# MeteoSwiss/topo-descriptors

Measured on AMD Instinct MI355X. Metric: Mpixels/s (and % HBM roofline) per descriptor, 1/2/4/8 MI355X, higher is better.
Workload: dtype f32

## Files before the change

topo_descriptors_amd/csrc/disc_ring_wide_impl.hpp:

```cpp
#pragma once

#include "wide_classify.hpp"

namespace topo {

namespace {

constexpr int NCW = 6;

template <int SIZE>
struct WGeo {
    static constexpr DiscTable<SIZE> T = make_disc_table<SIZE>();
    static_assert(T.centre == 0 && T.off_min == -T.off_max, "odd disc sizes only");
    static constexpr int M = T.off_max;
    static constexpr int DL = (M + NCW - 1) / NCW;
    static constexpr int NVL = 64 - 2 * DL;
    static constexpr int TILE_W = NCW * NVL;
    static constexpr int X0 = NCW * DL;
    static constexpr int W = 64 * NCW;
    static constexpr int NR = T.num_runs;
    static_assert(NVL >= 16, "disc too wide for one wavefront");
    struct Sched {
        int first_step[SIZE];
        int order[SIZE];
        int centre_run;
    };
    static constexpr Sched make() {
        Sched t{};
        for (int r = 0; r < SIZE; ++r) t.first_step[r] = -1;
        for (int r = 0; r < SIZE; ++r) t.order[r] = 0;
        t.centre_run = -1;
        for (int D = 0; D <= DL; ++D)
            for (int s = 0; s < NCW; ++s)
                for (int q = 0; q < NCW; ++q) {
                    const int dr = NCW * D + s - q, dl = -NCW * D + s - q;
                    if (dr >= 0 && dr <= M) {
                        const int r = T.run_of[dr - T.off_min];
                        if (D > t.first_step[r]) t.first_step[r] = D;
                    }
                    if (dl < 0 && dl >= -M) {
                        const int r = T.run_of[dl - T.off_min];
                        if (D > t.first_step[r]) t.first_step[r] = D;
                    }
                }
        int n = 0;
        for (int D = DL; D >= 0; --D)
            for (int d = M; d >= 0; --d) {
                const int r = T.run_of[d - T.off_min];
                bool seen = false;
                for (int i = 0; i < n; ++i) seen = seen || t.order[i] == r;
                if (!seen && t.first_step[r] == D) t.order[n++] = r;
            }
        for (int r = 0; r < NR; ++r)
            if (T.run_lo[r] == 0 && T.run_hi[r] == 0) t.centre_run = r;
        return t;
    }
    static constexpr Sched S = make();
    static_assert(S.centre_run >= 0, "the disc's outermost column is the pixel's own row");
};

template <int SIZE>
struct WideCfg {
    using G = WGeo<SIZE>;
    static constexpr int SW = 3;
    static constexpr int CW = 8;
    static constexpr int NW = SW + CW;
    static constexpr int RPW = 2;
    static constexpr int B = CW * RPW;
    static constexpr int TH = 64;
    static constexpr int PPT = TH / B;
    static constexpr int R = SIZE + 2 * B;
    static constexpr int GR = 6;
    static constexpr int HALO = SIZE - 1;
    static constexpr int PAD = 1 + (B - (1 + HALO + B) % B) % B;
    static constexpr int PRO = PAD + HALO + B;
    static constexpr int NB_PRO = PRO / B;
    static constexpr size_t LDS = (size_t)(R + GR) * G::W * sizeof(uint32_t) + 2 * SW * sizeof(int) + 16;
    static_assert(SW * 128 == G::W, "two staged columns per staging lane");
    static_assert(TH % B == 0 && PRO % B == 0, "whole batches");
    static_assert(LDS <= 160 * 1024, "ring does not fit LDS");
    static_assert(NB_PRO <= 15, "batch history: two fields of a flag word");
};

constexpr bool tpi_wide_ring_fits(int size) {
    return size >= 5 && size % 2 == 1 && (size_t)(size + 32 + 6) * 384 * 4 + 64 <= 160 * 1024 && 64 - 2 * ((size / 2 + 5) / 6) >= 16;
}

template <int SIZE, int GR>
struct WPair {
    using G = WGeo<SIZE>;
    static constexpr int NR = G::NR;
    static constexpr int NK = 2 * G::M + 3;
    struct Tab {
        int rows;
        int nb;
        int kb[NK];
        int first[NK];
        int base[NK];
        int use[SIZE][2][2];
        int nload[SIZE];
        int load[SIZE][4];
    };
    static constexpr Tab make() {
        Tab t{};
        bool need[NK] = {};
        for (int i = 0; i < NR; ++i) {
            const int r = G::S.order[i];
            for (int w = 0; w < 2; ++w) {
                t.use[i][w][0] = G::T.run_hi[r] + 1 + G::M + w;
                t.use[i][w][1] = G::T.run_lo[r] + G::M + w;
            }
            for (int w = 0; w < 2; ++w)
                for (int e = 0; e < 2; ++e) {
                    const int k = t.use[i][w][e];
                    if (!need[k]) t.load[i][t.nload[i]++] = k;
                    need[k] = true;
                }
        }
        for (int k = 0; k < NK; ++k) {
            if (!need[k]) continue;
            ++t.rows;
            if (t.nb == 0 || k > t.kb[t.nb - 1] + GR) t.kb[t.nb++] = k;
            t.base[k] = t.nb - 1;
        }
        for (int b = 0; b < t.nb; ++b) t.first[b] = NR;
        for (int i = NR - 1; i >= 0; --i)
            for (int n = 0; n < t.nload[i]; ++n) t.first[t.base[t.load[i][n]]] = i;
        return t;
    }
    static constexpr Tab T = make();
    static constexpr bool check() {
        bool loaded[NK] = {};
        for (int i = 0; i < NR; ++i) {
            for (int n = 0; n < T.nload[i]; ++n) {
                const int k = T.load[i][n], b = T.base[k];
                if (k < T.kb[b] || k - T.kb[b] > GR || T.first[b] > i || loaded[k]) return false;
                loaded[k] = true;
            }
            for (int w = 0; w < 2; ++w)
                for (int e = 0; e < 2; ++e)
                    if (!loaded[T.use[i][w][e]]) return false;
        }
        return true;
    }
    static constexpr int kUnshared = 4 * NR;
    static_assert(check(), "every row loaded once, before its uses, within GR rows of a base formed by then");
    static_assert(T.rows < kUnshared, "the pair shares no prefix row");
    static_assert(SIZE != 67 || T.rows == 55, "67 px: 55 distinct prefix rows a pair (84 unshared)");
};

template <int N, int I = 0, class F>
__device__ __forceinline__ void wide_static_for(F&& f) {
    if constexpr (I < N) {
        f(std::integral_constant<int, I>{});
        wide_static_for<N, I + 1>(f);
    }
}

template <int SIZE>
struct WSweep {
    using G = WGeo<SIZE>;
    struct Tab {
        int firstR[G::DL + 1][NCW], firstL[G::DL + 1][NCW];
        int lo_s[G::NR][2][G::DL + 1][NCW], hi_s[G::NR][2][G::DL + 1][NCW];
    };
    static constexpr int tap(int side, int D, int s, int t) { return (side == 0 ? NCW * D : -NCW * D) + s - t; }
    static constexpr bool takes(int side, int di) { return side == 0 ? di >= 0 && di <= G::M : di < 0 && di >= -G::M; }
    static constexpr Tab make() {
        Tab t{};
        for (int D = 0; D <= G::DL; ++D)
            for (int o = 0; o < NCW; ++o) t.firstR[D][o] = t.firstL[D][o] = -1;
        for (int j = G::NR - 1; j >= 0; --j)
            for (int s = NCW - 1; s >= 0; --s)
                for (int D = 0; D <= G::DL; ++D)
                    for (int o = 0; o < NCW; ++o) {
                        const int dr = NCW * D + s - o, dl = -NCW * D + s - o;
                        if (dr >= 0 && dr <= G::M && G::T.run_of[dr - G::T.off_min] == G::S.order[j]) t.firstR[D][o] = j * NCW + s;
                        if (dl < 0 && dl >= -G::M && G::T.run_of[dl - G::T.off_min] == G::S.order[j]) t.firstL[D][o] = j * NCW + s;
                    }
        for (int j = 0; j < G::NR; ++j)
            for (int side = 0; side < 2; ++side)
                for (int D = 0; D <= G::DL; ++D)
                    for (int o = 0; o < NCW; ++o) {
                        int lo = NCW, hi = -1;
                        for (int s = 0; s < NCW; ++s) {
                            const int di = tap(side, D, s, o);
                            if (takes(side, di) && G::T.run_of[di - G::T.off_min] == G::S.order[j]) {
                                lo = s < lo ? s : lo;
                                hi = s;
                            }
                        }
                        t.lo_s[j][side][D][o] = lo;
                        t.hi_s[j][side][D][o] = hi;
                    }
        return t;
    }
    static constexpr Tab T = make();
    static constexpr bool covers() {
        int hits[NCW][2 * G::M + 1] = {};
        int total = 0;
        for (int j = 0; j < G::NR; ++j)
            for (int side = 0; side < 2; ++side)
                for (int D = 0; D <= G::DL; ++D)
                    for (int o = 0; o < NCW; ++o)
                        for (int s = T.lo_s[j][side][D][o]; s <= T.hi_s[j][side][D][o]; ++s) {
                            const int di = tap(side, D, s, o);
                            if (di < -G::M || di > G::M) return false;
                            ++hits[o][di + G::M];
                            ++total;
                        }
        for (int o = 0; o < NCW; ++o)
            for (int d = 0; d <= 2 * G::M; ++d)
                if (hits[o][d] != 1) return false;
        return total == NCW * (2 * G::M + 1);
    }
    static constexpr bool firsts_start_intervals() {
        for (int side = 0; side < 2; ++side)
            for (int D = 0; D <= G::DL; ++D)
                for (int o = 0; o < NCW; ++o) {
                    const int f = side == 0 ? T.firstR[D][o] : T.firstL[D][o];
                    for (int j = 0; j < G::NR; ++j) {
                        const bool empty = T.lo_s[j][side][D][o] > T.hi_s[j][side][D][o];
                        if (f < 0 || j < f / NCW) {
                            if (!empty) return false;
                        } else if (j == f / NCW) {
                            if (empty || T.lo_s[j][side][D][o] != f % NCW) return false;
                        }
                    }
                }
        return true;
    }
    static_assert(covers(), "the intervals take every tap of every output once: SIZE taps an output");
    static_assert(SIZE != 67 || NCW * (2 * G::M + 1) == 402, "67 px: 402 taps per side pair");
    static_assert(firsts_start_intervals(), "firstR / firstL name an interval's first column");
    static constexpr int prio_of(int D) { return 3 - (G::DL - D) * 4 / (G::DL + 1); }
};

#ifndef WIDE_LEAD
#define WIDE_LEAD 2
#endif
#ifndef WIDE_PRIO
#define WIDE_PRIO 1
#endif

#ifndef WIDE_STAMPS
#define WIDE_STAMPS 0
#endif
#ifndef WIDE_LEAN
#define WIDE_LEAN 1
#endif
#ifndef WIDE_STAGE_CEILING
#define WIDE_STAGE_CEILING 0
#endif
#if WIDE_STAMPS
constexpr int kWideStampBlocks = 2, kWideStampWaves = 11, kWideStampFields = 5;
__device__ unsigned long long wide_stamps[kWideStampBlocks][kWideStampWaves][kWideStampFields];
__device__ __forceinline__ uint32_t wide_now() {
    const uint32_t t = (uint32_t)__builtin_amdgcn_s_memtime();
    asm volatile("s_waitcnt lgkmcnt(0)" ::: "memory");
    return t;
}
#endif

typedef uint32_t u32x2w __attribute__((ext_vector_type(2)));
typedef __attribute__((address_space(3))) const char lds_char;
typedef __attribute__((address_space(1))) const u32x2w glb_u32x2w;
typedef __attribute__((address_space(3))) const volatile u32x2w lds_u32x2w;

template <int SIZE, int R, int GR, int LEAD, bool PRIO>
__device__ __forceinline__ void wide_pair_sum(const uint32_t* ring, int s0, int lane, uint32_t (&acc)[2][NCW], uint32_t (&ctr)[2][NCW]) {
    using G = WGeo<SIZE>;
    using PT = WPair<SIZE, GR>;
    using SW_ = WSweep<SIZE>;
    constexpr int NR = G::NR;
    constexpr int DL = G::DL;
    constexpr int M = G::M;
    constexpr uint32_t PB = (uint32_t)G::W * 4;
    constexpr uint32_t RB = (uint32_t)R * PB;
    u32x2w row[PT::NK][3];
    uint32_t pR[2][DL + 1][NCW], pL[2][DL + 1][NCW];
    uint32_t aR[2][NCW], aL[2][NCW];
    uint32_t vb[PT::T.nb];
    lds_char* q = (lds_char*)ring;
    const uint32_t b0 = (uint32_t)s0 * PB, lb = (uint32_t)lane * (NCW * 4);
    auto fetch = [&](auto I) {
        constexpr int i = decltype(I)::value;
#pragma unroll
        for (int b = 0; b < PT::T.nb; ++b)
            if (PT::T.first[b] == i) {
                const uint32_t d = b0 + (uint32_t)PT::T.kb[b] * PB;
                vb[b] = lb + min(d, d - RB);
                asm("" : "+v"(vb[b]));
            }
#pragma unroll
        for (int n = 0; n < PT::T.nload[i]; ++n) {
            const int k = PT::T.load[i][n];
            lds_char* pk = q + vb[PT::T.base[k]] + (uint32_t)(k - PT::T.kb[PT::T.base[k]]) * PB;
#pragma unroll
            for (int h = 0; h < 3; ++h) row[k][h] = *(lds_u32x2w*)(pk + 8 * h);
        }
    };
    auto close = [&](auto DD) {
        constexpr int D = decltype(DD)::value;
        wide_static_for<NCW * 2>([&](auto TW) {
            constexpr int t = decltype(TW)::value / 2, w = decltype(TW)::value % 2;
            constexpr bool anyr = SW_::T.firstR[D][t] >= 0, anyl = SW_::T.firstL[D][t] >= 0;
            uint32_t pr = 0, pl = 0;
            if constexpr (anyr) pr = pR[w][D][t];
            if constexpr (anyl) pl = pL[w][D][t];
            if constexpr (D == DL) {
                aR[w][t] = pr;
                aL[w][t] = pl;
            } else if constexpr (D == 0) {
                uint32_t own = anyr && anyl ? pr + pl : anyr ? pr : pl;
                asm("" : "+v"(own));
                own = hop_up(aL[w][t]) + own;
                asm("" : "+v"(own));
                aR[w][t] = hop(aR[w][t]) + own;
                asm("" : "+v"(aR[w][t]));
            } else {
                if constexpr (anyr) {
                    asm("" : "+v"(pr));
                    aR[w][t] = hop(aR[w][t]) + pr;
                } else {
                    aR[w][t] = hop(aR[w][t]);
                }
                if constexpr (anyl) {
                    asm("" : "+v"(pl));
                    aL[w][t] = hop_up(aL[w][t]) + pl;
                } else {
                    aL[w][t] = hop_up(aL[w][t]);
                }
            }
        });
        RING_SB();
    };
    wide_static_for<(LEAD < NR ? LEAD : NR)>([&](auto I) { fetch(I); });
    if constexpr (PRIO) CHAIN_SETPRIO(3);
    static_assert(DL >= 1 && G::S.first_step[G::S.order[0]] == DL, "the first run opens the chains, the last step (D = 0) closes both");
    wide_static_for<NR>([&](auto J) {
        constexpr int j = decltype(J)::value;
        constexpr int r = G::S.order[j];
        constexpr int D = G::S.first_step[r];
        constexpr int Dprev = j == 0 ? DL : G::S.first_step[G::S.order[j > 0 ? j - 1 : 0]];
        constexpr int Dnext = j + 1 < NR ? G::S.first_step[G::S.order[j + 1 < NR ? j + 1 : j]] : -1;
        if constexpr (PRIO && SW_::prio_of(D) != SW_::prio_of(Dprev)) CHAIN_SETPRIO(SW_::prio_of(D));
        if constexpr (j + LEAD < NR) fetch(std::integral_constant<int, j + LEAD>{});
        RING_SB();
        uint32_t cv[2][NCW], pre[2][NCW], suf[2][NCW];
#pragma unroll
        for (int w = 0; w < 2; ++w) {
#pragma unroll
            for (int s = 0; s < NCW; ++s) {
                cv[w][s] = row[PT::T.use[j][w][0]][s / 2][s % 2] - row[PT::T.use[j][w][1]][s / 2][s % 2];
                if (r == G::S.centre_run) ctr[w][s] = cv[w][s];
            }
            pre[w][0] = cv[w][0];
            suf[w][NCW - 1] = cv[w][NCW - 1];
#pragma unroll
            for (int s = 1; s < NCW; ++s) {
                pre[w][s] = pre[w][s - 1] + cv[w][s];
                suf[w][NCW - 1 - s] = suf[w][NCW - s] + cv[w][NCW - 1 - s];
            }
        }
        wide_static_for<2 * (DL + 1) * NCW>([&](auto ET) {
            constexpr int side = decltype(ET)::value / ((DL + 1) * NCW);
            constexpr int E = decltype(ET)::value / NCW % (DL + 1), t = decltype(ET)::value % NCW;
            constexpr int a = SW_::T.lo_s[j][side][E][t], b = SW_::T.hi_s[j][side][E][t];
            if constexpr (a <= b) {
                static_assert(E <= D, "a run arrives at the first step that takes it");
                constexpr bool starts = (side == 0 ? SW_::T.firstR[E][t] : SW_::T.firstL[E][t]) / NCW == j;
#pragma unroll
                for (int w = 0; w < 2; ++w) {
                    const uint32_t iv = a == b ? cv[w][a] : a == 0 ? pre[w][b] : b == NCW - 1 ? suf[w][a] :
                                        b == a + 1 ? cv[w][a] + cv[w][b] : pre[w][b] - pre[w][a - 1];
                    uint32_t& acc_p = side == 0 ? pR[w][E][t] : pL[w][E][t];
                    acc_p = starts ? iv : acc_p + iv;
                }
            }
        });
        RING_SB();
        wide_static_for<D - Dnext>([&](auto C) { close(std::integral_constant<int, D - decltype(C)::value>{}); });
    });
#pragma unroll
    for (int w = 0; w < 2; ++w)
#pragma unroll
        for (int t = 0; t < NCW; ++t) acc[w][t] = aR[w][t];
}


template <int SIZE>
__global__ __launch_bounds__(WideCfg<SIZE>::NW * 64) void tpi_ring_wide_kernel(WaveArgs p, int tiles_x, int tiles_y, PartRun deal) {
    using G = WGeo<SIZE>;
    using C = WideCfg<SIZE>;
    constexpr int B = C::B, R = C::R, PPT = C::PPT, SW = C::SW, NB_PRO = C::NB_PRO, DL = G::DL;
    constexpr unsigned kWindow = (1u << NB_PRO) - 1u;
    constexpr int kBad = 1, kFracOnly = 1 << 15;
    constexpr unsigned kHistMask = kWindow | kWindow * kFracOnly;
    extern __shared__ __attribute__((aligned(16))) uint32_t lds_u[];
    uint32_t* Q = lds_u;
    int* wflags = reinterpret_cast<int*>(Q + (R + C::GR) * G::W);

    const int nb = (int)gridDim.x;
    const int vb = (nb & 7) ? (int)blockIdx.x : (int)(blockIdx.x & 7) * (nb >> 3) + (int)(blockIdx.x >> 3);
    const int lane = threadIdx.x & 63;
    const int wave = __builtin_amdgcn_readfirstlane((int)(threadIdx.x >> 6));
    const int ntiles = tiles_x * tiles_y;
    const int first = deal.first(vb);
    const int last = min(first + deal.count(vb), ntiles);
    const double inv_nm1 = 1.0 / ((double)G::T.taps - 1.0);
    const int rmin = max(0, p.in_row0), rmax = min(p.gny, p.in_row0 + p.in_rows);
    const bool stager = wave < SW;
    const int scol = 128 * wave + 2 * lane;
    int seen_tiles = 0, seen_frac = 0;
#if WIDE_STAMPS
    uint32_t ts_n = 0, ts_all = 0, ts_drain = 0, ts_bar = 0, ts_pair = 0, ts_prev = 0;
#endif

#pragma unroll 1
    for (int pos = first; pos < last;) {
        const int tile0 = pos;
        const int ty0 = tile0 % tiles_y;
        const int run_tiles = min(last - tile0, tiles_y - ty0);
        const int strip = tile0 / tiles_y;
        const int nphase = run_tiles * PPT;
        const int ox0 = strip * G::TILE_W;
        const int oyS = (p.out_row0 / C::TH + ty0) * C::TH;
        const int gx0 = ox0 - G::X0;
        const int gy0 = oyS - G::M - C::PAD;
        const int gcol = gx0 + scol;
        const bool col_ok = stager && gcol >= 0 && gcol < p.nx;
        const float* src = p.in + (col_ok ? gcol : 0);
        constexpr bool kLean = WIDE_LEAN || WIDE_STAGE_CEILING;
        const bool cols_in = kLean && __builtin_amdgcn_ballot_w64(col_ok) == ~0ull;
        const uint32_t voff = (uint32_t)(col_ok ? gcol : 0) * 4u;
        auto load_batch = [&](int n0, float2 (&v)[B]) {
            const int g0 = gy0 + n0;
            if (kLean && g0 >= rmin && g0 + B <= rmax && p.nx < (1 << 29)) {
                uint64_t rowa = reinterpret_cast<uint64_t>(p.in) + (uint64_t)(g0 - p.in_row0) * (uint64_t)p.nx * sizeof(float);
                uint32_t vo = voff;
                asm("" : "+v"(vo));
#pragma unroll
                for (int r = 0; r < B; ++r) {
                    asm("" : "+s"(rowa));
                    const u32x2w t = *reinterpret_cast<glb_u32x2w*>(rowa + vo);
                    v[r] = make_float2(__uint_as_float(t.x), __uint_as_float(t.y));
                    rowa += (uint64_t)p.nx * sizeof(float);
                }
                asm volatile("");
                return;
            }
#pragma unroll
            for (int r = 0; r < B; ++r) {
                int gy = g0 + r;
                gy = min(max(gy, rmin), rmax - 1);
                v[r] = *reinterpret_cast<const float2*>(src + (size_t)(gy - p.in_row0) * p.nx);
            }
        };
        uint32_t run0 = 0, run1 = 0;
        int wslot = 0;
        auto stage_batch = [&](int n0, const float2 (&v)[B]) {
            WideClassAcc cls;
            auto take = [&](float x0, float x1) {
                const int i0 = (int)x0, i1 = (int)x1;
#if !WIDE_STAGE_CEILING
                wide_classify_row(cls, x0, x1);
#endif
                run0 += (uint32_t)i0;
                run1 += (uint32_t)i1;
                const u32x2w v2 = {run0, run1};
                return v2;
            };
            const int g0 = gy0 + n0;
            if (cols_in && g0 >= rmin && g0 + B <= rmax && wslot + B <= R) {
                uint32_t* q = Q + wslot * G::W + scol;
#pragma unroll
                for (int r = 0; r < B; ++r) *reinterpret_cast<u32x2w*>(q + r * G::W) = take(v[r].x, v[r].y);
            } else {
#pragma unroll
                for (int r = 0; r < B; ++r) {
                    const int gy = g0 + r;
                    const bool ok = col_ok && gy >= rmin && gy < rmax;
                    int sl = wslot + r;
                    sl = sl >= R ? sl - R : sl;
                    *reinterpret_cast<u32x2w*>(Q + sl * G::W + scol) = take(ok ? v[r].x : 0.0f, ok ? v[r].y : 0.0f);
                }
            }
            const int glo = wslot < C::GR ? wslot : 0;
            const int ghi = wslot < C::GR ? C::GR : min(wslot + B - R, C::GR);
            if (glo < ghi) {
#pragma unroll
                for (int g = 0; g < C::GR; ++g) {
                    const int sl = min(max(g, glo), ghi - 1);
                    *reinterpret_cast<u32x2w*>(Q + (sl + R) * G::W + scol) = *reinterpret_cast<const u32x2w*>(Q + sl * G::W + scol);
                }
            }
#if WIDE_STAGE_CEILING
            return 0;
#else
            return wide_classify_batch(cls, kAbsLim + 1.0f, kBad, kFracOnly);
#endif
        };
        auto advance_wslot = [&]() {
            wslot += B;
            wslot = wslot >= R ? wslot - R : wslot;
        };
        unsigned hist = 0;
        auto fold = [&](int parity) {
            int all = 0;
#pragma unroll
            for (int w = 0; w < SW; ++w) all |= wflags[parity * SW + w];
            all = __builtin_amdgcn_readfirstlane(all);
            hist = ((hist << 1) | (unsigned)all) & kHistMask;
        };

        const int ocol = gx0 + lane * NCW;
        const bool lane_ok = lane >= DL && lane < DL + G::NVL && ocol < p.nx;
        __syncthreads();
        auto run_phases = [&](auto STG) {
        constexpr bool stg = decltype(STG)::value;
        float2 va[stg ? B : 1];
        if constexpr (stg) {
            int bits = 0;
#pragma unroll 1
            for (int k = 0; k < NB_PRO; ++k) {
                load_batch(k * B, va);
                bits |= stage_batch(k * B, va) << (NB_PRO - 1 - k);
                advance_wslot();
            }
            if (lane == 0) wflags[wave] = bits;
            load_batch(C::PRO, va);
        } else {
            for (int k = 0; k < NB_PRO; ++k) advance_wslot();
        }
        __syncthreads();
        {
            int all = 0;
#pragma unroll
            for (int w = 0; w < SW; ++w) all |= wflags[w];
            hist = (unsigned)__builtin_amdgcn_readfirstlane(all) & kHistMask;
        }

        bool tile_frac = false;
#pragma unroll 1
        for (int ph = 0; ph < nphase; ++ph) {
            const bool compute = (hist & kWindow) == 0;
            const int oyA = oyS + ph * B;
            tile_frac = tile_frac || (hist & (kWindow * kFracOnly)) != 0;
            if (!compute) {
                const int r0 = max(oyA, p.out_row0), r1 = min(oyA + B, p.out_row0 + p.out_rows) - 1;
                if (r0 <= r1 && threadIdx.x == 0) {
                    const int base = p.out_row0 / p.map_th;
                    const int mx0 = ox0 / p.map_tw, mx1 = (min(ox0 + G::TILE_W, p.nx) - 1) / p.map_tw;
                    for (int mx = mx0; mx <= mx1; ++mx)
                        for (int my = r0 / p.map_th; my <= r1 / p.map_th; ++my) p.defer[mx * p.map_tiles_y + (my - base)] = kNeedsFraction;
                }
            }
            if (ph % PPT == PPT - 1) {
                ++seen_tiles;
                seen_frac += tile_frac ? 1 : 0;
                tile_frac = false;
            }
            if constexpr (stg) {
                if constexpr (WIDE_PRIO != 0) CHAIN_SETPRIO(3);
                const int seen = stage_batch(C::PRO + ph * B, va);
                if (lane == 0) wflags[((ph + 1) & 1) * SW + wave] = seen;
                if constexpr (WIDE_PRIO != 0) CHAIN_SETPRIO(0);
                load_batch(C::PRO + (ph + 1) * B, va);
            } else if (compute) {
                static_assert(C::RPW == 2, "a chain wave sums its two rows of a phase in one sweep");
                const int j = (wave - SW) * C::RPW;
                const int oy = oyA + j;
                if (oy + C::RPW > p.out_row0 && oy < p.out_row0 + p.out_rows) {
                    const int s0 = (C::PAD - 1 + ph * B + j) % R;
                    uint32_t acc[C::RPW][NCW], ctr[C::RPW][NCW];
                    wide_pair_sum<SIZE, R, C::GR, WIDE_LEAD, WIDE_PRIO != 0>(Q, s0, lane, acc, ctr);
#pragma unroll
                    for (int k = 0; k < C::RPW; ++k) {
                        const bool row_ok = oy + k >= p.out_row0 && oy + k < p.out_row0 + p.out_rows;
                        if (lane_ok && row_ok) {
                            float* o = p.tpi + (size_t)(oy + k - p.out_row0) * p.nx + ocol;
                            float out_t[NCW];
#pragma unroll
                            for (int t = 0; t < NCW; ++t) {
                                const int xi = (int)ctr[k][t];
                                out_t[t] = (float)((double)xi - (double)((int)acc[k][t] - xi) * inv_nm1);
                            }
#pragma unroll
                            for (int P = 0; P < NCW / 2; ++P)
                                if (ocol + 2 * P < p.nx) *reinterpret_cast<float2*>(o + 2 * P) = make_float2(out_t[2 * P], out_t[2 * P + 1]);
                        }
                    }
                }
            }
            advance_wslot();
#if WIDE_STAMPS
            const uint32_t t0 = wide_now();
            if constexpr (!stg && WIDE_STAMPS == 1) asm volatile("s_waitcnt vmcnt(0)" ::: "memory");
            const uint32_t t1 = wide_now();
#endif
            __syncthreads();
#if WIDE_STAMPS
            const uint32_t t2 = wide_now(), t3 = wide_now();
            if (ph > 0) {
                ts_n += 1;
                ts_all += t2 - ts_prev;
                ts_drain += t1 - t0;
                ts_bar += t2 - t1;
                ts_pair += t3 - t2;
            }
            ts_prev = t2;
#endif
            fold((ph + 1) & 1);
        }
        if constexpr (stg) {
#pragma unroll
            for (int r = 0; r < B; ++r) asm volatile("" ::"v"(va[r].x), "v"(va[r].y));
        }
        };
        if (stager) run_phases(std::true_type{});
        else run_phases(std::false_type{});
        pos += run_tiles;
    }
#if WIDE_STAMPS
    static_assert(WideCfg<SIZE>::NW == kWideStampWaves, "one record per wave");
    if (lane == 0 && (vb == 0 || vb == nb / 2)) {
        unsigned long long* o = wide_stamps[vb == 0 ? 0 : 1][wave];
        o[0] = (unsigned long long)ts_n, o[1] = (unsigned long long)ts_all, o[2] = (unsigned long long)ts_drain;
        o[3] = (unsigned long long)ts_bar, o[4] = (unsigned long long)ts_pair;
    }
#endif
    if (p.report != nullptr && vb == nb / 2 && threadIdx.x == 0) {
        __hip_atomic_store(p.report + 1, (uint32_t)seen_frac, __ATOMIC_RELAXED, __HIP_MEMORY_SCOPE_SYSTEM);
        __hip_atomic_store(p.report, (uint32_t)seen_tiles, __ATOMIC_RELAXED, __HIP_MEMORY_SCOPE_SYSTEM);
    }
}

template <int SIZE>
int launch_ring_wide(const Block& b, float* tpi_out, int map_th, int map_tw) {
    using G = WGeo<SIZE>;
    using C = WideCfg<SIZE>;
    Context& c = ctx();
    TOPO_REQUIRE(c.seams.n == 0, "the wide ring takes single-block calls only");
    WaveArgs a = wave_args(b, tpi_out, nullptr);
    a.report = dem_memo_report(b);
    static int blocks_per_cu = 0;
    const auto clear_map = [&](WaveParts& ps, long) -> int {
        TOPO_REQUIRE(ps.n == 1 && ps.a[0].map_th == map_th && ps.a[0].map_tw == map_tw, "wide ring: tile map of another geometry");
        const size_t map_bytes = (size_t)((b.nx + map_tw - 1) / map_tw) * ps.a[0].map_tiles_y;
        TOPO_HIP(hipMemsetAsync(ps.a[0].defer, kTileDone, map_bytes, c.compute));
        return TOPO_AMD_OK;
    };
    return launch_tiles(tpi_ring_wide_kernel<SIZE>, nullptr, &blocks_per_cu, C::NW * 64, C::LDS, 0, b, a, C::TH, G::TILE_W, true, false,
                        map_th, map_tw, clear_map);
}

}

}
```

Before: 352,000.

## Prefetch next phase's lead LDS rows before the barrier and widen stored columns

```diff
diff --git a/topo_descriptors_amd/csrc/disc_ring_wide_impl.hpp b/topo_descriptors_amd/csrc/disc_ring_wide_impl.hpp
--- a/topo_descriptors_amd/csrc/disc_ring_wide_impl.hpp
+++ b/topo_descriptors_amd/csrc/disc_ring_wide_impl.hpp
@@ -15,9 +15,10 @@
     static constexpr int M = T.off_max;
     static constexpr int DL = (M + NCW - 1) / NCW;
     static constexpr int NVL = 64 - 2 * DL;
-    static constexpr int TILE_W = NCW * NVL;
-    static constexpr int X0 = NCW * DL;
     static constexpr int W = 64 * NCW;
+    static constexpr int XV = (M + 1) / 2 * 2;
+    static constexpr int TILE_W = W - 2 * XV;
+    static constexpr int X0 = XV;
     static constexpr int NR = T.num_runs;
     static_assert(NVL >= 16, "disc too wide for one wavefront");
     struct Sched {
@@ -143,6 +144,24 @@
         }
         return true;
     }
+    static constexpr int lead_rows(int lead) {
+        int n = 0;
+        for (int i = 0; i < lead && i < NR; ++i) n += T.nload[i];
+        return n;
+    }
+    static constexpr int lead_bases(int lead) {
+        int n = 0;
+        for (int b = 0; b < T.nb; ++b) n += T.first[b] < lead ? 1 : 0;
+        return n;
+    }
+    static constexpr int lead_reach(int lead) {
+        int m = 0;
+        for (int i = 0; i < lead && i < NR; ++i)
+            for (int n = 0; n < T.nload[i]; ++n) m = T.load[i][n] > m ? T.load[i][n] : m;
+        return m;
+    }
+    template <int LEAD, int B>
+    static constexpr bool lead_is_published() { return lead_reach(LEAD) + B - 2 <= 2 * G::M; }
     static constexpr int kUnshared = 4 * NR;
     static_assert(check(), "every row loaded once, before its uses, within GR rows of a base formed by then");
     static_assert(T.rows < kUnshared, "the pair shares no prefix row");
@@ -230,7 +249,21 @@
                 }
         return true;
     }
+    static constexpr bool edges_valid() {
+        for (int c = G::XV; c < G::W - G::XV; ++c) {
+            const int lane = c / NCW, o = c % NCW;
+            if (c - G::M < 0 || c + G::M > G::W - 1) return false;
+            for (int D = 0; D <= G::DL; ++D) {
+                if (lane + D > 63 && T.firstR[D][o] >= 0) return false;
+                if (lane - D < 0 && T.firstL[D][o] >= 0) return false;
+            }
+        }
+        return true;
+    }
     static_assert(covers(), "the intervals take every tap of every output once: SIZE taps an output");
+    static_assert(G::XV % 2 == 0 && G::XV >= G::M && G::TILE_W % 2 == 0,
+                  "whole store pairs, a disc's reach inside the staged columns");
+    static_assert(edges_valid(), "a stored column takes nothing from beyond the wave's ends");
     static_assert(SIZE != 67 || NCW * (2 * G::M + 1) == 402, "67 px: 402 taps per side pair");
     static_assert(firsts_start_intervals(), "firstR / firstL name an interval's first column");
     static constexpr int prio_of(int D) { return 3 - (G::DL - D) * 4 / (G::DL + 1); }
@@ -243,6 +276,10 @@
 #define WIDE_PRIO 1
 #endif
 
+#ifndef WIDE_BOUNDARY
+#define WIDE_BOUNDARY 0
+#endif
+
 #ifndef WIDE_STAMPS
 #define WIDE_STAMPS 0
 #endif
@@ -253,7 +290,7 @@
 #define WIDE_STAGE_CEILING 0
 #endif
 #if WIDE_STAMPS
-constexpr int kWideStampBlocks = 2, kWideStampWaves = 11, kWideStampFields = 5;
+constexpr int kWideStampBlocks = 2, kWideStampWaves = 11, kWideStampFields = 7;
 __device__ unsigned long long wide_stamps[kWideStampBlocks][kWideStampWaves][kWideStampFields];
 __device__ __forceinline__ uint32_t wide_now() {
     const uint32_t t = (uint32_t)__builtin_amdgcn_s_memtime();
@@ -267,39 +304,87 @@
 typedef __attribute__((address_space(1))) const u32x2w glb_u32x2w;
 typedef __attribute__((address_space(3))) const volatile u32x2w lds_u32x2w;
 
-template <int SIZE, int R, int GR, int LEAD, bool PRIO>
-__device__ __forceinline__ void wide_pair_sum(const uint32_t* ring, int s0, int lane, uint32_t (&acc)[2][NCW], uint32_t (&ctr)[2][NCW]) {
+template <int SIZE, int R, int GR, int I>
+__device__ __forceinline__ void wide_pair_fetch(const uint32_t* ring, uint32_t b0, uint32_t lb,
+                                                u32x2w (&row)[WPair<SIZE, GR>::NK][3], uint32_t (&vb)[WPair<SIZE, GR>::T.nb]) {
+    using PT = WPair<SIZE, GR>;
+    constexpr uint32_t PB = (uint32_t)WGeo<SIZE>::W * 4;
+    constexpr uint32_t RB = (uint32_t)R * PB;
+    lds_char* q = (lds_char*)ring;
+#pragma unroll
+    for (int b = 0; b < PT::T.nb; ++b)
+        if (PT::T.first[b] == I) {
+            const uint32_t d = b0 + (uint32_t)PT::T.kb[b] * PB;
+            vb[b] = lb + min(d, d - RB);
+            asm("" : "+v"(vb[b]));
+        }
+#pragma unroll
+    for (int n = 0; n < PT::T.nload[I]; ++n) {
+        const int k = PT::T.load[I][n];
+        lds_char* pk = q + vb[PT::T.base[k]] + (uint32_t)(k - PT::T.kb[PT::T.base[k]]) * PB;
+#pragma unroll
+        for (int h = 0; h < 3; ++h) row[k][h] = *(lds_u32x2w*)(pk + 8 * h);
+    }
+}
+
+template <int SIZE, int GR, int LEAD, bool OUT, class ROWS, class BASES>
+__device__ __forceinline__ void wide_lead_rows(ROWS& lrow, BASES& lvb, u32x2w (&row)[WPair<SIZE, GR>::NK][3],
+                                               uint32_t (&vb)[WPair<SIZE, GR>::T.nb]) {
+    using PT = WPair<SIZE, GR>;
+    int n = 0;
+#pragma unroll
+    for (int i = 0; i < LEAD && i < PT::NR; ++i)
+#pragma unroll
+        for (int m = 0; m < PT::T.nload[i]; ++m, ++n)
+#pragma unroll
+            for (int h = 0; h < 3; ++h) {
+                if (OUT) lrow[n][h] = row[PT::T.load[i][m]][h];
+                else row[PT::T.load[i][m]][h] = lrow[n][h];
+            }
+    int nb = 0;
+#pragma unroll
+    for (int b = 0; b < PT::T.nb; ++b)
+        if (PT::T.first[b] < LEAD) {
+            if (OUT) lvb[nb] = vb[b];
+            else vb[b] = lvb[nb];
+            ++nb;
+        }
+}
+
+template <int SIZE, int R, int GR, int LEAD>
+__device__ __forceinline__ void wide_pair_lead(const uint32_t* ring, uint32_t b0, int lane,
+                                               u32x2w (&lrow)[WPair<SIZE, GR>::lead_rows(LEAD)][3],
+                                               uint32_t (&lvb)[WPair<SIZE, GR>::lead_bases(LEAD)]) {
+    using PT = WPair<SIZE, GR>;
+    constexpr int NR = WGeo<SIZE>::NR;
+    const uint32_t lb = (uint32_t)lane * (NCW * 4);
+    u32x2w row[PT::NK][3];
+    uint32_t vb[PT::T.nb];
+    wide_static_for<(LEAD < NR ? LEAD : NR)>(
+        [&](auto I) { wide_pair_fetch<SIZE, R, GR, decltype(I)::value>(ring, b0, lb, row, vb); });
+    wide_lead_rows<SIZE, GR, LEAD, true>(lrow, lvb, row, vb);
+}
+
+template <int SIZE, int R, int GR, int LEAD, bool PRIO, bool LEAD_DONE>
+__device__ __forceinline__ void wide_pair_sum(const uint32_t* ring, uint32_t b0, int lane,
+                                              u32x2w (&lrow)[WPair<SIZE, GR>::lead_rows(LEAD)][3],
+                                              uint32_t (&lvb)[WPair<SIZE, GR>::lead_bases(LEAD)], uint32_t (&acc)[2][NCW],
+                                              uint32_t (&ctr)[2][NCW]
+#if WIDE_STAMPS
+                                              , uint32_t& t_sweep
+#endif
+) {
     using G = WGeo<SIZE>;
     using PT = WPair<SIZE, GR>;
     using SW_ = WSweep<SIZE>;
     constexpr int NR = G::NR;
     constexpr int DL = G::DL;
-    constexpr int M = G::M;
-    constexpr uint32_t PB = (uint32_t)G::W * 4;
-    constexpr uint32_t RB = (uint32_t)R * PB;
-    u32x2w row[PT::NK][3];
     uint32_t pR[2][DL + 1][NCW], pL[2][DL + 1][NCW];
     uint32_t aR[2][NCW], aL[2][NCW];
+    u32x2w row[PT::NK][3];
     uint32_t vb[PT::T.nb];
-    lds_char* q = (lds_char*)ring;
-    const uint32_t b0 = (uint32_t)s0 * PB, lb = (uint32_t)lane * (NCW * 4);
-    auto fetch = [&](auto I) {
-        constexpr int i = decltype(I)::value;
-#pragma unroll
-        for (int b = 0; b < PT::T.nb; ++b)
-            if (PT::T.first[b] == i) {
-                const uint32_t d = b0 + (uint32_t)PT::T.kb[b] * PB;
-                vb[b] = lb + min(d, d - RB);
-                asm("" : "+v"(vb[b]));
-            }
-#pragma unroll
-        for (int n = 0; n < PT::T.nload[i]; ++n) {
-            const int k = PT::T.load[i][n];
-            lds_char* pk = q + vb[PT::T.base[k]] + (uint32_t)(k - PT::T.kb[PT::T.base[k]]) * PB;
-#pragma unroll
-            for (int h = 0; h < 3; ++h) row[k][h] = *(lds_u32x2w*)(pk + 8 * h);
-        }
-    };
+    const uint32_t lb = (uint32_t)lane * (NCW * 4);
+    auto fetch = [&](auto I) { wide_pair_fetch<SIZE, R, GR, decltype(I)::value>(ring, b0, lb, row, vb); };
     auto close = [&](auto DD) {
         constexpr int D = decltype(DD)::value;
         wide_static_for<NCW * 2>([&](auto TW) {
@@ -335,7 +420,11 @@
         });
         RING_SB();
     };
-    wide_static_for<(LEAD < NR ? LEAD : NR)>([&](auto I) { fetch(I); });
+    if constexpr (LEAD_DONE) wide_lead_rows<SIZE, GR, LEAD, false>(lrow, lvb, row, vb);
+    else wide_static_for<(LEAD < NR ? LEAD : NR)>([&](auto I) { fetch(I); });
+#if WIDE_STAMPS
+    t_sweep = wide_now();
+#endif
     if constexpr (PRIO) CHAIN_SETPRIO(3);
     static_assert(DL >= 1 && G::S.first_step[G::S.order[0]] == DL, "the first run opens the chains, the last step (D = 0) closes both");
     wide_static_for<NR>([&](auto J) {
@@ -393,7 +482,7 @@
 __global__ __launch_bounds__(WideCfg<SIZE>::NW * 64) void tpi_ring_wide_kernel(WaveArgs p, int tiles_x, int tiles_y, PartRun deal) {
     using G = WGeo<SIZE>;
     using C = WideCfg<SIZE>;
-    constexpr int B = C::B, R = C::R, PPT = C::PPT, SW = C::SW, NB_PRO = C::NB_PRO, DL = G::DL;
+    constexpr int B = C::B, R = C::R, PPT = C::PPT, SW = C::SW, NB_PRO = C::NB_PRO;
     constexpr unsigned kWindow = (1u << NB_PRO) - 1u;
     constexpr int kBad = 1, kFracOnly = 1 << 15;
     constexpr unsigned kHistMask = kWindow | kWindow * kFracOnly;
@@ -414,7 +503,7 @@
     const int scol = 128 * wave + 2 * lane;
     int seen_tiles = 0, seen_frac = 0;
 #if WIDE_STAMPS
-    uint32_t ts_n = 0, ts_all = 0, ts_drain = 0, ts_bar = 0, ts_pair = 0, ts_prev = 0;
+    uint32_t ts_n = 0, ts_all = 0, ts_drain = 0, ts_bar = 0, ts_pair = 0, ts_prev = 0, ts_nsw = 0, ts_lead = 0;
 #endif
 
 #pragma unroll 1
@@ -506,16 +595,27 @@
             wslot = wslot >= R ? wslot - R : wslot;
         };
         unsigned hist = 0;
-        auto fold = [&](int parity) {
+        auto fold = [&](int parity, auto AT_ONCE) {
+            int f[SW];
+#pragma unroll
+            for (int w = 0; w < SW; ++w) f[w] = wflags[parity * SW + w];
+            static_assert(SW == 3, "the flag words of the staging waves, held at once");
+            if constexpr (decltype(AT_ONCE)::value) asm("" : "+v"(f[0]), "+v"(f[1]), "+v"(f[2]));
             int all = 0;
 #pragma unroll
-            for (int w = 0; w < SW; ++w) all |= wflags[parity * SW + w];
+            for (int w = 0; w < SW; ++w) all |= f[w];
             all = __builtin_amdgcn_readfirstlane(all);
             hist = ((hist << 1) | (unsigned)all) & kHistMask;
         };
 
         const int ocol = gx0 + lane * NCW;
-        const bool lane_ok = lane >= DL && lane < DL + G::NVL && ocol < p.nx;
+        bool pair_ok[NCW / 2];
+        bool lane_ok = false;
+#pragma unroll
+        for (int P = 0; P < NCW / 2; ++P) {
+            pair_ok[P] = lane * NCW + 2 * P >= G::XV && lane * NCW + 2 * P < G::W - G::XV && ocol + 2 * P < p.nx;
+            lane_ok = lane_ok || pair_ok[P];
+        }
         __syncthreads();
         auto run_phases = [&](auto STG) {
         constexpr bool stg = decltype(STG)::value;
@@ -540,6 +640,43 @@
             for (int w = 0; w < SW; ++w) all |= wflags[w];
             hist = (unsigned)__builtin_amdgcn_readfirstlane(all) & kHistMask;
         }
+
+        using PT = WPair<SIZE, C::GR>;
+        constexpr uint32_t PB = (uint32_t)G::W * 4, RB = (uint32_t)R * PB;
+        constexpr bool kAhead = !stg && WIDE_BOUNDARY != 0;
+        static_assert(C::RPW == 2, "a chain wave sums its two rows of a phase in one sweep");
+        static_assert(!kAhead || PT::template lead_is_published<WIDE_LEAD, B>(),
+                      "the lead fetches read rows published a barrier earlier");
+        static_assert(C::PAD - 1 + B - C::RPW < R, "a run's first slots need no wrap");
+        const int pj = stg ? 0 : (wave - SW) * C::RPW;
+        [[maybe_unused]] int py = oyS + pj;
+        [[maybe_unused]] long long prow = (long long)(py - p.out_row0) * p.nx;
+        [[maybe_unused]] uint32_t pb0 = (uint32_t)(C::PAD - 1 + pj) * PB;
+        [[maybe_unused]] u32x2w row[PT::lead_rows(WIDE_LEAD)][3];
+        [[maybe_unused]] uint32_t vbase[PT::lead_bases(WIDE_LEAD)];
+        if constexpr (kAhead) {
+            if (nphase > 0) wide_pair_lead<SIZE, R, C::GR, WIDE_LEAD>(Q, pb0, lane, row, vbase);
+        }
+#if WIDE_STAMPS
+        [[maybe_unused]] uint32_t t_sweep = 0;
+#endif
+        [[maybe_unused]] auto store_row = [&](bool row_ok, long long off, const uint32_t (&acc_k)[NCW],
+                                              const uint32_t (&ctr_k)[NCW]) {
+            if (lane_ok && row_ok) {
+                float out_t[NCW];
+#pragma unroll
+                for (int t = 0; t < NCW; ++t) {
+                    const int xi = (int)ctr_k[t];
+                    out_t[t] = (float)((double)xi - (double)((int)acc_k[t] - xi) * inv_nm1);
+                }
+#pragma unroll
+                for (int t = 0; t < NCW; ++t) asm volatile("" : "+v"(out_t[t]));
+#pragma unroll
+                for (int P = 0; P < NCW / 2; ++P)
+                    if (__builtin_expect(pair_ok[P], true))
+                        *reinterpret_cast<float2*>(p.tpi + (off + ocol + 2 * P)) = make_float2(out_t[2 * P], out_t[2 * P + 1]);
+            }
+        };
 
         bool tile_frac = false;
 #pragma unroll 1
@@ -568,28 +705,39 @@
                 if constexpr (WIDE_PRIO != 0) CHAIN_SETPRIO(0);
                 load_batch(C::PRO + (ph + 1) * B, va);
             } else if (compute) {
-                static_assert(C::RPW == 2, "a chain wave sums its two rows of a phase in one sweep");
-                const int j = (wave - SW) * C::RPW;
-                const int oy = oyA + j;
-                if (oy + C::RPW > p.out_row0 && oy < p.out_row0 + p.out_rows) {
-                    const int s0 = (C::PAD - 1 + ph * B + j) % R;
-                    uint32_t acc[C::RPW][NCW], ctr[C::RPW][NCW];
-                    wide_pair_sum<SIZE, R, C::GR, WIDE_LEAD, WIDE_PRIO != 0>(Q, s0, lane, acc, ctr);
-#pragma unroll
-                    for (int k = 0; k < C::RPW; ++k) {
-                        const bool row_ok = oy + k >= p.out_row0 && oy + k < p.out_row0 + p.out_rows;
-                        if (lane_ok && row_ok) {
-                            float* o = p.tpi + (size_t)(oy + k - p.out_row0) * p.nx + ocol;
-                            float out_t[NCW];
-#pragma unroll
-                            for (int t = 0; t < NCW; ++t) {
-                                const int xi = (int)ctr[k][t];
-                                out_t[t] = (float)((double)xi - (double)((int)acc[k][t] - xi) * inv_nm1);
-                            }
-#pragma unroll
-                            for (int P = 0; P < NCW / 2; ++P)
-                                if (ocol + 2 * P < p.nx) *reinterpret_cast<float2*>(o + 2 * P) = make_float2(out_t[2 * P], out_t[2 * P + 1]);
-                        }
+                if constexpr (kAhead) {
+                    if (py + C::RPW > p.out_row0 && py < p.out_row0 + p.out_rows) {
+                        uint32_t acc[C::RPW][NCW], ctr[C::RPW][NCW];
+                        wide_pair_sum<SIZE, R, C::GR, WIDE_LEAD, WIDE_PRIO != 0, true>(Q, pb0, lane, row, vbase, acc, ctr
+#if WIDE_STAMPS
+                                                                                       , t_sweep
+#endif
+                        );
+#pragma unroll
+                        for (int k = 0; k < C::RPW; ++k)
+                            store_row(py + k >= p.out_row0 && py + k < p.out_row0 + p.out_rows, prow + (long long)k * p.nx,
+                                      acc[k], ctr[k]);
+#if WIDE_STAMPS
+                        if (ph > 0) ts_nsw += 1, ts_lead += t_sweep - ts_prev;
+#endif
+                    }
+                } else {
+                    const int oy = oyA + pj;
+                    if (oy + C::RPW > p.out_row0 && oy < p.out_row0 + p.out_rows) {
+                        const int s0 = (C::PAD - 1 + ph * B + pj) % R;
+                        uint32_t acc[C::RPW][NCW], ctr[C::RPW][NCW];
+                        wide_pair_sum<SIZE, R, C::GR, WIDE_LEAD, WIDE_PRIO != 0, false>(Q, (uint32_t)s0 * PB, lane, row, vbase, acc, ctr
+#if WIDE_STAMPS
+                                                                                        , t_sweep
+#endif
+                        );
+#pragma unroll
+                        for (int k = 0; k < C::RPW; ++k)
+                            store_row(oy + k >= p.out_row0 && oy + k < p.out_row0 + p.out_rows, (long long)(oy + k - p.out_row0) * p.nx,
+                                      acc[k], ctr[k]);
+#if WIDE_STAMPS
+                        if (ph > 0) ts_nsw += 1, ts_lead += t_sweep - ts_prev;
+#endif
                     }
                 }
             }
@@ -599,7 +747,25 @@
             if constexpr (!stg && WIDE_STAMPS == 1) asm volatile("s_waitcnt vmcnt(0)" ::: "memory");
             const uint32_t t1 = wide_now();
 #endif
-            __syncthreads();
+            if constexpr (kAhead) {
+                py += B;
+                prow += (long long)B * p.nx;
+                pb0 += (uint32_t)B * PB;
+                pb0 = pb0 >= RB ? pb0 - RB : pb0;
+                if (ph + 1 < nphase) {
+                    wide_pair_lead<SIZE, R, C::GR, WIDE_LEAD>(Q, pb0, lane, row, vbase);
+                } else {
+#pragma unroll
+                    for (int n = 0; n < PT::lead_rows(WIDE_LEAD); ++n)
+#pragma unroll
+                        for (int h = 0; h < 3; ++h) asm volatile("" : "=v"(row[n][h]));
+#pragma unroll
+                    for (int b = 0; b < PT::lead_bases(WIDE_LEAD); ++b) asm volatile("" : "=v"(vbase[b]));
+                }
+                asm volatile("s_barrier" ::: "memory");
+            } else {
+                __syncthreads();
+            }
 #if WIDE_STAMPS
             const uint32_t t2 = wide_now(), t3 = wide_now();
             if (ph > 0) {
@@ -611,7 +777,7 @@
             }
             ts_prev = t2;
 #endif
-            fold((ph + 1) & 1);
+            fold((ph + 1) & 1, std::bool_constant<kAhead>{});
         }
         if constexpr (stg) {
 #pragma unroll
@@ -628,6 +794,7 @@
         unsigned long long* o = wide_stamps[vb == 0 ? 0 : 1][wave];
         o[0] = (unsigned long long)ts_n, o[1] = (unsigned long long)ts_all, o[2] = (unsigned long long)ts_drain;
         o[3] = (unsigned long long)ts_bar, o[4] = (unsigned long long)ts_pair;
+        o[5] = (unsigned long long)ts_nsw, o[6] = (unsigned long long)ts_lead;
     }
 #endif
     if (p.report != nullptr && vb == nb / 2 && threadIdx.x == 0) {
```

New measurement: 358,400, median of 6. +1.8%, better.
